# yongxuUSTC/DNN-for-speech-enhancement

Hardware: AMD Instinct MI355X
Metric: training frames/sec (257x11 input, 3x2048 DNN) (higher is better)
Workload: dtype f32; 1 GPU; C2: 2827->2048->2048->2048->257 ReLU+dropout(0.1/0.2), fp32, 256 frames/GPU/step (global bunch 256), lrate 1, momentum 0.5, 102400-frame chunk resident in HBM; parallelism=dp1, global_bunch=256, exchange=none, launcher=single process

## Files before the change

dnn-for-speech-enhancement_amd/csrc/bp_kernels.h:

```cpp
#pragma once
#include <hip/hip_runtime.h>
#include <stddef.h>
#include <stdint.h>

#include "bp_device.h"

enum { EPI_FWD_HIDDEN = 0, EPI_FWD_OUT = 1, EPI_DGRAD = 2, EPI_WGRAD_UPDATE = 3, EPI_WGRAD_STORE = 4,
       EPI_OUT_SPLIT = 6 ,
       EPI_FWD_OUT_LOGI = 7, EPI_OUT_SPLIT_LOGI = 8 };
static constexpr bool epi_out(int epi) { return epi == EPI_FWD_OUT || epi == EPI_FWD_OUT_LOGI; }
static constexpr bool epi_out_split(int epi) { return epi == EPI_OUT_SPLIT || epi == EPI_OUT_SPLIT_LOGI; }
static constexpr int OUT_SPLITS = 4;

struct GemmArgs {
    const float *A, *B;
    int lda, ldb;
    int K;
    int tiles_m, tiles_n;
#ifdef BP_TRACE
    unsigned long long *trace;
#endif
    int k_split;
    size_t slab_stride;
    float *ks_slab; unsigned *ks_ticket;
};

struct EpiArgs {
    float *C; int ldc;
    int m_limit, n_limit;
    int n_true;
    const float *bias;
    float alpha;
    int act;
    const float *aux; int ldaux;
    int lin_cols;
    float *aux2; int ldaux2;
    union {
        float scale;
        float rdiv;
    };
    float mom, c1, wc, ndiv;
    float *bias_w, *bias_d, *bias_g;
    uint32_t drop_thresh, seed_lo, seed_hi, step, layer;
    int frame_off;
    const uint8_t *mask; int ldmask;
    int loss;
    unsigned *done;
};
static_assert(sizeof(EpiArgs) == 160 && offsetof(EpiArgs, aux2) == 56 && offsetof(EpiArgs, done) == 152, "lin_cols / loss must sit in padding");
static_assert(offsetof(EpiArgs, rdiv) == 68 && offsetof(EpiArgs, scale) == 68 && offsetof(EpiArgs, mom) == 72 && offsetof(EpiArgs, ndiv) == 84,
              "rdiv lies in scale's word, in front of mom, c1, wc, ndiv");
typedef __attribute__((address_space(1))) const float *GlobalOperand;
#define BP_PIN_OPERANDS(g, ...) do { GlobalOperand pa_ = (GlobalOperand)(g).A, pb_ = (GlobalOperand)(g).B;                                \
        asm volatile("" : "+s"(pa_), "+s"(pb_), "+s"((g).lda), "+s"((g).ldb), "+s"((g).K), "+s"((g).tiles_m), "+s"((g).tiles_n), ##__VA_ARGS__); \
        (g).A = (const float *)pa_; (g).B = (const float *)pb_; } while (0)
__device__ __forceinline__ GemmArgs operand_args(const GemmArgs &s)
{
    GemmArgs g{};
    g.A = s.A; g.B = s.B; g.lda = s.lda; g.ldb = s.ldb; g.K = s.K; g.tiles_m = s.tiles_m; g.tiles_n = s.tiles_n;
    return g;
}

struct EpiPre { float bias; f32x16 p0, p1; };

template <class T>
__device__ __forceinline__ T *uniform_ptr(T *p)
{
    const unsigned long long v = (unsigned long long)p;
    const unsigned lo = __builtin_amdgcn_readfirstlane((unsigned)v), hi = __builtin_amdgcn_readfirstlane((unsigned)(v >> 32));
    typedef __attribute__((address_space(1))) T *GlobalPtr;
    return (T *)(GlobalPtr)(((unsigned long long)hi << 32) | lo);
}

template <class T>
__device__ __forceinline__ T *sgpr_row_base(T *p)
{
    typedef __attribute__((address_space(1))) T *GlobalPtr;
    GlobalPtr q = (GlobalPtr)p;
    asm volatile("" : "+s"(q));
    return (T *)q;
}

template <int EPI, int R0, int RN>
__device__ __forceinline__ void epilogue_fetch(const EpiArgs &e, int mb, int nb, int lane, EpiPre &p)
{
    if constexpr (EPI == EPI_WGRAD_UPDATE) {
        const int mbc = mb < e.m_limit ? mb : 0;
        const float *cw = uniform_ptr(e.C + (size_t)mbc * e.ldc + nb);
        const float *cd = uniform_ptr(e.aux2 + (size_t)mbc * e.ldc + nb);
        const unsigned ldc = __builtin_amdgcn_readfirstlane(e.ldc);
        const unsigned lob = 4u * ((unsigned)(4 * (lane >> 5)) * (unsigned)e.ldc + (unsigned)(lane & 31));
#pragma unroll
        for (int r = R0; r < R0 + RN; ++r) {
            const unsigned ro = (unsigned)((r & 3) + 8 * (r >> 2)) * ldc;
            p.p0[r] = *reinterpret_cast<const float *>(reinterpret_cast<const char *>(sgpr_row_base(cw + ro)) + lob);
            p.p1[r] = *reinterpret_cast<const float *>(reinterpret_cast<const char *>(sgpr_row_base(cd + ro)) + lob);
        }
        return;
    }
    const int n = nb + (lane & 31);
    const int rbase = mb + 4 * (lane >> 5);
    static_assert(!epi_out_split(EPI), "fetched as EPI_FWD_OUT[_LOGI]");
    if constexpr (EPI == EPI_FWD_HIDDEN || epi_out(EPI)) p.bias = e.bias[n];
    if constexpr (epi_out(EPI) || EPI == EPI_DGRAD) {
        if (epi_out(EPI) && !e.C) return;
#pragma unroll
        for (int r = R0; r < R0 + RN; ++r) {
            const int m = rbase + (r & 3) + 8 * (r >> 2);
            const int mc = m < e.m_limit ? m : e.m_limit - 1;
            p.p0[r] = e.aux[(size_t)mc * e.ldaux + n];
        }
    }
}

template <int R0, int RN>
__device__ __forceinline__ void block_store(const EpiArgs &e, int mb, int nb, int lane, const float (&v)[RN])
{
    if (mb + 32 <= e.m_limit) {
        float *c = uniform_ptr(e.C + (size_t)mb * e.ldc + nb);
        const unsigned ldc = __builtin_amdgcn_readfirstlane(e.ldc);
        const unsigned lob = 4u * ((unsigned)(4 * (lane >> 5)) * (unsigned)e.ldc + (unsigned)(lane & 31));
#pragma unroll
        for (int r = R0; r < R0 + RN; ++r) {
            const unsigned ro = (unsigned)((r & 3) + 8 * (r >> 2)) * ldc;
            *reinterpret_cast<float *>(reinterpret_cast<char *>(sgpr_row_base(c + ro)) + lob) = v[r - R0];
        }
        return;
    }
    const int n = nb + (lane & 31), rbase = mb + 4 * (lane >> 5);
#pragma unroll
    for (int r = R0; r < R0 + RN; ++r) {
        const int m = rbase + (r & 3) + 8 * (r >> 2);
        if (m < e.m_limit) e.C[(size_t)m * e.ldc + n] = v[r - R0];
    }
}

template <int EPI, int R0, int RN, bool RCP = false>
__device__ __forceinline__ void epilogue_block(const EpiArgs &e, int mb, int nb, const f32x16 &acc, int lane,
                                               const EpiPre &p)
{
    static_assert(!RCP || EPI == EPI_WGRAD_UPDATE, "only the fused update divides");
    static_assert(RN % 4 == 0 && R0 % 4 == 0, "register range must cover whole 4-row groups");
    if constexpr (EPI == EPI_WGRAD_UPDATE || EPI == EPI_WGRAD_STORE) {
        const int n = nb + (lane & 31);
        if (n >= e.n_limit || mb >= e.m_limit) return;
        float *cw = uniform_ptr(e.C + (size_t)mb * e.ldc + nb);
        const unsigned ldc = __builtin_amdgcn_readfirstlane(e.ldc);
        const unsigned lob = 4u * ((unsigned)(4 * (lane >> 5)) * (unsigned)e.ldc + (unsigned)(lane & 31));
#pragma unroll
        for (int r = R0; r < R0 + RN; ++r) {
            const unsigned ro = (unsigned)((r & 3) + 8 * (r >> 2)) * ldc;
            if constexpr (EPI == EPI_WGRAD_UPDATE) {
                float *cd = uniform_ptr(e.aux2 + (size_t)mb * e.ldc + nb);
                const float w = p.p0[r];
                const float d = update_delta<RCP>(e.mom, e.c1, e.wc, e.ndiv, e.rdiv, p.p1[r], acc[r], w);
                *reinterpret_cast<float *>(reinterpret_cast<char *>(sgpr_row_base(cd + ro)) + lob) = d;
                *reinterpret_cast<float *>(reinterpret_cast<char *>(sgpr_row_base(cw + ro)) + lob) = d + 1.0f * w;
            } else {
                __hip_atomic_store(reinterpret_cast<float *>(reinterpret_cast<char *>(sgpr_row_base(cw + ro)) + lob), acc[r], __ATOMIC_RELAXED, __HIP_MEMORY_SCOPE_SYSTEM);
            }
        }
        return;
    }
    const int n = nb + (lane & 31);
    const int rbase = mb + 4 * (lane >> 5);
    if (n >= e.n_limit) return;
    if constexpr (EPI == EPI_FWD_HIDDEN) {
        const float bn = p.bias;
        const bool live = n < e.n_true;
        float y[RN];
#pragma unroll
        for (int q = R0 / 4; q < (R0 + RN) / 4; ++q) {
            uint32_t w[4] = {0xFFFFFFFFu, 0xFFFFFFFFu, 0xFFFFFFFFu, 0xFFFFFFFFu};
            const int r0 = rbase + 8 * q;
            if (e.mask) {
#pragma unroll
                for (int j = 0; j < 4; ++j) w[j] = (r0 + j < e.m_limit && live && e.mask[(size_t)(r0 + j) * e.ldmask + n]) ? 0u : 0xFFFFFFFFu;
            } else if (e.drop_thresh) drop_words4(w, r0, n, e.frame_off, (uint32_t)e.n_true, e.layer, e.step, e.seed_lo, e.seed_hi);
#pragma unroll
            for (int j = 0; j < 4; ++j) {
                y[q * 4 + j - R0] = act_fwd(e.act, e.alpha * acc[q * 4 + j] + bn);
                if (!live || w[j] < e.drop_thresh) y[q * 4 + j - R0] = 0.0f;
            }
        }
        block_store<R0, RN>(e, mb, nb, lane, y);
    } else if constexpr (EPI == EPI_FWD_OUT) {
        const float bn = p.bias;
        const bool live = n < e.n_true;
#pragma unroll
        for (int r = R0; r < R0 + RN; ++r) {
            const int m = rbase + (r & 3) + 8 * (r >> 2);
            if (m < e.m_limit) {
                const float o = live ? e.alpha * acc[r] + bn : 0.0f;
                if (e.aux2) e.aux2[(size_t)m * e.ldaux2 + n] = o;
                if (e.C) e.C[(size_t)m * e.ldc + n] = live ? e.scale * (o - p.p0[r]) : 0.0f;
            }
        }
    } else if constexpr (EPI == EPI_FWD_OUT_LOGI) {
        const float bn = p.bias;
        const bool live = n < e.n_true, logi = live && n >= e.lin_cols, chain = logi && e.loss == 1;
#pragma unroll
        for (int r = R0; r < R0 + RN; ++r) {
            const int m = rbase + (r & 3) + 8 * (r >> 2);
            if (m < e.m_limit) {
                const float z = live ? e.alpha * acc[r] + bn : 0.0f;
                const float o = logi ? 1.0f / (1.0f + expf(-z)) : z;
                if (e.aux2) e.aux2[(size_t)m * e.ldaux2 + n] = o;
                if (e.C) {
                    float d = live ? e.scale * (o - p.p0[r]) : 0.0f;
                    if (chain) d *= o * (1.0f - o);
                    e.C[(size_t)m * e.ldc + n] = d;
                }
            }
        }
    } else if constexpr (EPI == EPI_DGRAD) {
        float d[RN];
#pragma unroll
        for (int r = R0; r < R0 + RN; ++r) d[r - R0] = act_bwd(e.act, p.p0[r]) * acc[r];
        block_store<R0, RN>(e, mb, nb, lane, d);
    } else {
        static_assert(EPI == EPI_WGRAD_UPDATE || EPI == EPI_WGRAD_STORE, "epilogue without a branch");
    }
}

template <bool RCP>
__device__ __forceinline__ void bias_update(const EpiArgs &e, int n, float s)
{
    const float d = update_delta<RCP>(e.mom, e.c1, 0.0f, e.ndiv, e.rdiv, e.bias_d[n], s, e.bias_w[n]);
    e.bias_d[n] = d;
    e.bias_w[n] = d + 1.0f * e.bias_w[n];
}

template <int R0>
__device__ __forceinline__ void out_split_store(const EpiArgs &e, float *slab, int mb, int nb, const f32x16 &acc, int lane)
{
    const int n = nb + (lane & 31), rbase = mb + 4 * (lane >> 5);
    if (n >= e.n_limit) return;
#pragma unroll
    for (int r = R0; r < R0 + 4; ++r) {
        const int m = rbase + (r & 3) + 8 * (r >> 2);
        if (m < e.m_limit) __hip_atomic_store(slab + (size_t)m * e.ldc + n, acc[r], __ATOMIC_RELAXED, __HIP_MEMORY_SCOPE_AGENT);
    }
}
template <int R0>
__device__ __forceinline__ void out_split_sum(const EpiArgs &e, const float *slab0, size_t stride, int mb, int nb, f32x16 &acc, int lane)
{
    const int n = nb + (lane & 31), rbase = mb + 4 * (lane >> 5);
    if (n >= e.n_limit) return;
    float p[OUT_SPLITS][4];
#pragma unroll
    for (int z = 0; z < OUT_SPLITS; ++z)
#pragma unroll
        for (int rr = 0; rr < 4; ++rr) {
            const int r = R0 + rr, m = rbase + (r & 3) + 8 * (r >> 2), mc = m < e.m_limit ? m : e.m_limit - 1;
            p[z][rr] = __hip_atomic_load(slab0 + z * stride + (size_t)mc * e.ldc + n, __ATOMIC_RELAXED, __HIP_MEMORY_SCOPE_AGENT);
        }
#pragma unroll
    for (int rr = 0; rr < 4; ++rr) {
        float s = p[0][rr];
#pragma unroll
        for (int z = 1; z < OUT_SPLITS; ++z) s += p[z][rr];
        acc[R0 + rr] = s;
    }
}

template <int KS, int KSI>
__device__ __forceinline__ void ksplit_give(const f32x16 &acc, float *red, int wq, int lane)
{
    constexpr int RN = 16 / KS;
#pragma unroll
    for (int o = 0; o < KS; ++o) {
        if (o == KSI) continue;
#pragma unroll
        for (int rr = 0; rr < RN; ++rr) red[(((wq * KS + o) * KS + KSI) * RN + rr) * 64 + lane] = acc[o * RN + rr];
    }
}
template <int KS, int KSI>
__device__ __forceinline__ void ksplit_take(f32x16 &acc, const float *red, int wq, int lane)
{
    constexpr int RN = 16 / KS;
#pragma unroll
    for (int src = 0; src < KS; ++src) {
        if (src == KSI) continue;
#pragma unroll
        for (int rr = 0; rr < RN; ++rr) acc[KSI * RN + rr] += red[(((wq * KS + KSI) * KS + src) * RN + rr) * 64 + lane];
    }
}

template <int NVA, int NVB>
struct TileRegs { float4 a[NVA]; float4 b[NVB]; };

template <int BM, int BN, int BK, int WM, int WN, bool A_KC, bool B_KC, int EPI>
struct GemmCfg {
    static constexpr int KS = 4 / (WM * WN);
    static constexpr int TM = BM / (WM * 32), TN = BN / (WN * 32);
    static constexpr int LDA_S = A_KC ? BM + 1 : BM;
    static constexpr int LDB_S = B_KC ? BN + 1 : BN;
    static constexpr int A_STAGE = (BK * LDA_S + 3) & ~3, B_STAGE = (BK * LDB_S + 3) & ~3;
    static constexpr int NVA = BM * BK / 4 / 256, NVB = BN * BK / 4 / 256;
    static constexpr int LPS = (BK / 4 < 8) ? BK / 4 : 8;
    static constexpr bool BIASG = (EPI == EPI_WGRAD_UPDATE || EPI == EPI_WGRAD_STORE);
    static_assert(WM * WN * KS == 4 && TM >= 1 && TN >= 1, "wave layout");
    static_assert(BK % (2 * KS) == 0 && BK % 4 == 0, "BK");
    static_assert(NVA >= 1 && NVB >= 1, "tile too small for 256 threads");
    using Regs = TileRegs<NVA, NVB>;

    static constexpr int NCH = (TM * TN == 1) ? 2 : 1;
    static constexpr int NK = BK / KS / 2;
    static constexpr int step_row(int ks, int s) { return ks * (BK / KS) + 2 * s; }
    static constexpr int step_chain(int s) { return s % NCH; }

    struct Offs { unsigned a[NVA]; unsigned b[NVB]; };
    static __device__ __forceinline__ unsigned lane_off(unsigned &off)
    {
        asm volatile("" : "+v"(off));
        return off;
    }
    static __device__ __forceinline__ void make_offs(Offs &o, const GemmArgs &g, int tid)
    {
#pragma unroll
        for (int i = 0; i < NVA; ++i) {
            const int f = tid + i * 256;
            if constexpr (A_KC) {
                const int l8 = f % LPS, seg = f / LPS, row = seg % BM, k4 = (seg / BM) * LPS + l8;
                o.a[i] = 4u * (unsigned)(row * g.lda + k4 * 4);
            } else {
                const int c4 = f % (BM / 4), k = f / (BM / 4);
                o.a[i] = 4u * (unsigned)(k * g.lda + c4 * 4);
            }
        }
#pragma unroll
        for (int i = 0; i < NVB; ++i) {
            const int f = tid + i * 256;
            if constexpr (B_KC) {
                const int l8 = f % LPS, seg = f / LPS, row = seg % BN, k4 = (seg / BN) * LPS + l8;
                o.b[i] = 4u * (unsigned)(row * g.ldb + k4 * 4);
            } else {
                const int c4 = f % (BN / 4), k = f / (BN / 4);
                o.b[i] = 4u * (unsigned)(k * g.ldb + c4 * 4);
            }
        }
    }
    static __device__ __forceinline__ const float *base_a(const GemmArgs &g, int m0, int k0)
    {
        return A_KC ? g.A + (size_t)m0 * g.lda + k0 : g.A + (size_t)k0 * g.lda + m0;
    }
    static __device__ __forceinline__ const float *base_b(const GemmArgs &g, int n0, int k0)
    {
        return B_KC ? g.B + (size_t)n0 * g.ldb + k0 : g.B + (size_t)k0 * g.ldb + n0;
    }
    static __device__ __forceinline__ void load_a(Regs &r, int i, const float *pa, Offs &o)
    {
        r.a[i] = *reinterpret_cast<const float4 *>(reinterpret_cast<const char *>(pa) + lane_off(o.a[i]));
    }
    static __device__ __forceinline__ void load_b(Regs &r, int i, const float *pb, Offs &o)
    {
        r.b[i] = *reinterpret_cast<const float4 *>(reinterpret_cast<const char *>(pb) + lane_off(o.b[i]));
    }
    static __device__ __forceinline__ void load(Regs &r, const float *pa, const float *pb, Offs &o)
    {
#pragma unroll
        for (int i = 0; i < NVA; ++i) load_a(r, i, pa, o);
#pragma unroll
        for (int i = 0; i < NVB; ++i) load_b(r, i, pb, o);
    }

    static __device__ __forceinline__ void store_a(const Regs &r, int i, float *As, int tid, int krows)
    {
        const int f = tid + i * 256;
        float4 v = r.a[i];
        if constexpr (BIASG && !A_KC) {
            if (f / (BM / 4) >= krows) v = make_float4(0.f, 0.f, 0.f, 0.f);
        }
        if constexpr (A_KC) {
            const int l8 = f % LPS, seg = f / LPS, row = seg % BM, k4 = (seg / BM) * LPS + l8;
            As[(k4 * 4 + 0) * LDA_S + row] = v.x; As[(k4 * 4 + 1) * LDA_S + row] = v.y;
            As[(k4 * 4 + 2) * LDA_S + row] = v.z; As[(k4 * 4 + 3) * LDA_S + row] = v.w;
        } else {
            const int c4 = f % (BM / 4), k = f / (BM / 4);
            *reinterpret_cast<float4 *>(As + k * LDA_S + c4 * 4) = v;
        }
    }
    static __device__ __forceinline__ void store_b(const Regs &r, int i, float *Bs, int tid, float4 &bsum)
    {
        const int f = tid + i * 256;
        const float4 v = r.b[i];
        if constexpr (B_KC) {
            const int l8 = f % LPS, seg = f / LPS, row = seg % BN, k4 = (seg / BN) * LPS + l8;
            Bs[(k4 * 4 + 0) * LDB_S + row] = v.x; Bs[(k4 * 4 + 1) * LDB_S + row] = v.y;
            Bs[(k4 * 4 + 2) * LDB_S + row] = v.z; Bs[(k4 * 4 + 3) * LDB_S + row] = v.w;
        } else {
            const int c4 = f % (BN / 4), k = f / (BN / 4);
            *reinterpret_cast<float4 *>(Bs + k * LDB_S + c4 * 4) = v;
            if constexpr (BIASG) {
                bsum.x += v.x; bsum.y += v.y; bsum.z += v.z; bsum.w += v.w;
            }
        }
    }
    static __device__ __forceinline__ void store(const Regs &r, float *As, float *Bs, int tid, float4 &bsum, int krows)
    {
#pragma unroll
        for (int i = 0; i < NVA; ++i) store_a(r, i, As, tid, krows);
#pragma unroll
        for (int i = 0; i < NVB; ++i) store_b(r, i, Bs, tid, bsum);
    }

    template <bool DO_STORE, bool DO_LOAD>
    static __device__ __forceinline__ void step(const float *As, const float *Bs, f32x16 (&acc)[NCH][TM][TN], int ks,
                                                int a_off, int b_off, int kh, const Regs &rs, float *AsN, float *BsN,
                                                Regs &rl, const float *pa, const float *pb, Offs &o, int tid,
                                                float4 &bsum, int krows)
    {
        constexpr int NP = NVA + NVB, RD = NK < 4 ? NK : 4;
        const float *ap = As + (step_row(ks, 0) + kh) * LDA_S + a_off;
        const float *bp = Bs + (step_row(ks, 0) + kh) * LDB_S + b_off;
        float av[NK][TM], bv[NK][TN];
        __builtin_amdgcn_sched_barrier(0);
#pragma unroll
        for (int s = 0; s < RD; ++s) {
#pragma unroll
            for (int i = 0; i < TM; ++i) av[s][i] = ap[step_row(0, s) * LDA_S + i * 32];
#pragma unroll
            for (int j = 0; j < TN; ++j) bv[s][j] = bp[step_row(0, s) * LDB_S + j * 32];
        }
        __builtin_amdgcn_sched_barrier(0);
        int pl = 0, ps = 0;
#pragma unroll
        for (int s = 0; s < NK; ++s) {
#pragma unroll
            for (int i = 0; i < TM; ++i)
#pragma unroll
                for (int j = 0; j < TN; ++j)
                    acc[step_chain(s)][i][j] = __builtin_amdgcn_mfma_f32_32x32x2f32(av[s][i], bv[s][j], acc[step_chain(s)][i][j], 0, 0, 0);
            if (s + RD < NK) {
#pragma unroll
                for (int i = 0; i < TM; ++i) av[s + RD][i] = ap[step_row(0, s + RD) * LDA_S + i * 32];
#pragma unroll
                for (int j = 0; j < TN; ++j) bv[s + RD][j] = bp[step_row(0, s + RD) * LDB_S + j * 32];
            }
            if constexpr (DO_LOAD) {
#pragma unroll
                for (int q = 0; q < NP; ++q) {
                    if (q == pl && (q * NK) / NP == s) {
                        if (q < NVA) load_a(rl, q, pa, o); else load_b(rl, q - NVA, pb, o);
                        ++pl;
                    }
                }
            }
            if constexpr (DO_STORE) {
#pragma unroll
                for (int q = 0; q < NP; ++q) {
                    if (q == ps && (q * NK) / NP == s) {
                        if (q < NVA) store_a(rs, q, AsN, tid, krows); else store_b(rs, q - NVA, BsN, tid, bsum);
                        ++ps;
                    }
                }
            }
            __builtin_amdgcn_sched_barrier(0);
        }
    }
};

template <bool M_SLOW>
__device__ __forceinline__ void xcd_tile(int b, int tiles_m, int tiles_n, int &tile_m, int &tile_n)
{
    if ((tiles_n & 7) == 0) {
        const int xcd = b & 7, j = b >> 3, per = tiles_n >> 3;
        if constexpr (M_SLOW) { tile_n = xcd * per + j % per; tile_m = j / per; }
        else { tile_n = xcd * per + j / tiles_m; tile_m = j % tiles_m; }
    } else { tile_m = b % tiles_m; tile_n = b / tiles_m; }
}
template <class Multi>
__device__ __forceinline__ int problem_of(const Multi &a, int b, int p)
{
    while (p + 1 < a.n && b >= a.first_tile[p + 1]) ++p;
    return p;
}

static inline bool covers_tiles(long long workgroups, const GemmArgs &g, int slices = 1)
{
    return g.tiles_m >= 0 && g.tiles_n >= 0 && workgroups >= (long long)g.tiles_m * g.tiles_n * slices;
}
template <class Multi>
static inline bool multi_covers_tiles(const Multi &a)
{
    if (a.n < 1 || a.n > 4) return false;
    for (int p = 0; p < a.n; ++p)
        if (!covers_tiles((long long)a.first_tile[p + 1] - a.first_tile[p], a.g[p])) return false;
    return true;
}

template <int BM, int BN, int BK, int WM, int WN, bool A_KC, bool B_KC, int EPI>
struct GemmKernel {
    using Cfg = GemmCfg<BM, BN, BK, WM, WN, A_KC, B_KC, EPI>;
    static constexpr int KS = Cfg::KS, TM = Cfg::TM, TN = Cfg::TN;
    static constexpr int A_STAGE = Cfg::A_STAGE, B_STAGE = Cfg::B_STAGE, STAGE = A_STAGE + B_STAGE;
    static constexpr bool BIASG = Cfg::BIASG;
    static constexpr int RED = (KS > 1) ? KS * WM * WN * 16 * 64 : 0;
    static constexpr int BIASRED = BIASG ? 256 / (BN / 4) * BN : 0;
    static constexpr int SMEM0 = (2 * STAGE > RED) ? 2 * STAGE : RED;
    static constexpr int SMEM = SMEM0 > BIASRED ? SMEM0 : BIASRED;
    static constexpr int MIN_WG = (SMEM * 4 > 80 * 1024) ? 1 : 2;

static __device__ __forceinline__ void run(const GemmArgs &g_in, const EpiArgs &e_in, int b, int block_y, float *smem)
{
    using Regs = typename Cfg::Regs;
    const int tid = threadIdx.x, lane = tid & 63, wave = __builtin_amdgcn_readfirstlane(tid >> 6);
    constexpr int EPI_E = EPI == EPI_OUT_SPLIT ? EPI_FWD_OUT : EPI == EPI_OUT_SPLIT_LOGI ? EPI_FWD_OUT_LOGI : EPI;
#ifdef BP_TRACE
#define TRACE(i) do { if (tid == 0 && g_in.trace) { g_in.trace[(size_t)b * 8 + (i)] = wall_clock64();           \
        if ((i) == 0) g_in.trace[(size_t)b * 8 + 6] = clock64();              \
        if ((i) == 3) g_in.trace[(size_t)b * 8 + 7] = clock64();           \
    } } while (0)
#else
#define TRACE(i) ((void)0)
#endif
#define K0_OF(t) (((t) * BK) < last_k0 ? ((t) * BK) : last_k0)
#define PA(t) Cfg::base_a(g, m0, K0_OF(t))
#define PB(t) Cfg::base_b(g, n0, K0_OF(t))
#define AS(buf) (smem + (buf) * STAGE)
#define BS(buf) (smem + (buf) * STAGE + A_STAGE)

    TRACE(0);
    GemmArgs g = operand_args(g_in);
    if constexpr (epi_out_split(EPI)) {
        const size_t kz = (size_t)block_y * g_in.k_split;
        g.A += A_KC ? kz : kz * g.lda;
        g.B += B_KC ? kz : kz * g.ldb;
    }
    BP_PIN_OPERANDS(g);
    const int tiles = g.tiles_m * g.tiles_n;
    if (b >= tiles) return;
    const int nt = (g.K + BK - 1) / BK, last_k0 = (nt - 1) * BK;
    typename Cfg::Offs offs;
    Cfg::make_offs(offs, g, tid);
    int tile_m, tile_n;
    xcd_tile<BIASG>(b, g.tiles_m, g.tiles_n, tile_m, tile_n);
    const int m0 = tile_m * BM, n0 = tile_n * BN;
    Regs r0, r1;
    Cfg::load(r0, PA(0), PB(0), offs);
    Cfg::load(r1, PA(1), PB(1), offs);
    __builtin_amdgcn_sched_barrier(0);

    int behind = 0;
    asm volatile("" : "+s"(behind));
    const EpiArgs e = *reinterpret_cast<const EpiArgs *>(reinterpret_cast<const char *>(&e_in) + behind);
    const int ks = wave / (WM * WN), wq = wave % (WM * WN), wm = wq / WN, wn = wq % WN;
    const int a_off = wm * TM * 32 + (lane & 31), b_off = wn * TN * 32 + (lane & 31);
    const int kh = lane >> 5;

    float4 bsum = make_float4(0.f, 0.f, 0.f, 0.f);
    const bool do_bias = BIASG && tile_m == 0;

    constexpr int NCH = Cfg::NCH;
    f32x16 accs[NCH][TM][TN];
#pragma unroll
    for (int c = 0; c < NCH; ++c)
#pragma unroll
        for (int i = 0; i < TM; ++i)
#pragma unroll
            for (int j = 0; j < TN; ++j)
#pragma unroll
                for (int r = 0; r < 16; ++r) accs[c][i][j][r] = 0.0f;

    EpiPre pre[TM][TN];
    const int mb0 = m0 + wm * TM * 32, nb0 = n0 + wn * TN * 32;
    if constexpr (KS == 1) {
#pragma unroll
        for (int i = 0; i < TM; ++i)
#pragma unroll
            for (int j = 0; j < TN; ++j) epilogue_fetch<EPI_E, 0, 16>(e, mb0 + i * 32, nb0 + j * 32, lane, pre[i][j]);
    } else {
        static_assert(KS == 1 || (TM == 1 && TN == 1), "in-workgroup k-split needs one block per wave");
        if (ks == 0) epilogue_fetch<EPI_E, 0, 16 / KS>(e, mb0, nb0, lane, pre[0][0]);
        if (ks == 1) epilogue_fetch<EPI_E, 16 / KS, 16 / KS>(e, mb0, nb0, lane, pre[0][0]);
        if constexpr (KS == 4) {
            if (ks == 2) epilogue_fetch<EPI_E, 8, 4>(e, mb0, nb0, lane, pre[0][0]);
            if (ks == 3) epilogue_fetch<EPI_E, 12, 4>(e, mb0, nb0, lane, pre[0][0]);
        }
    }

#define STEP(ST, LD, buf, RS, TS, RL, TL)                                                                  \
    Cfg::template step<ST, LD>(AS(buf), BS(buf), accs, ks, a_off, b_off, kh, RS, AS((buf) ^ 1), BS((buf) ^ 1),    \
                               RL, PA(TL), PB(TL), offs, tid, bsum, g.K - (TS) * BK)
    Cfg::store(r0, AS(0), BS(0), tid, bsum, g.K);
    __syncthreads();
    TRACE(1);
    int t = 0, buf = 0;
    if (__builtin_expect(nt >= 3, 1))
    for (; t + 3 <= nt; t += 2) {
        STEP(true, true, 0, r1, t + 1, r0, t + 2);
        __syncthreads();
        STEP(true, true, 1, r0, t + 2, r1, t + 3);
        __syncthreads();
    }
    if (nt - t == 2) {
        STEP(true, false, 0, r1, t + 1, r0, 0);
        __syncthreads();
        buf = 1;
    }
    STEP(false, false, buf, r0, 0, r0, 0);
    __syncthreads();
    TRACE(2);
#undef STEP
    __builtin_amdgcn_s_waitcnt(0x0F70);
    f32x16 (&acc)[TM][TN] = accs[0];
    if constexpr (NCH == 2) {
#pragma unroll
        for (int i = 0; i < TM; ++i)
#pragma unroll
            for (int j = 0; j < TN; ++j)
#pragma unroll
                for (int r = 0; r < 16; ++r) acc[i][j][r] += accs[1][i][j][r];
    }

    if constexpr (KS > 1) {
        if (ks == 0) ksplit_give<KS, 0>(acc[0][0], smem, wq, lane);
        if (ks == 1) ksplit_give<KS, 1>(acc[0][0], smem, wq, lane);
        if constexpr (KS == 4) {
            if (ks == 2) ksplit_give<KS, 2>(acc[0][0], smem, wq, lane);
            if (ks == 3) ksplit_give<KS, 3>(acc[0][0], smem, wq, lane);
        }
        __syncthreads();
        if (ks == 0) ksplit_take<KS, 0>(acc[0][0], smem, wq, lane);
        if (ks == 1) ksplit_take<KS, 1>(acc[0][0], smem, wq, lane);
        if constexpr (KS == 4) {
            if (ks == 2) ksplit_take<KS, 2>(acc[0][0], smem, wq, lane);
            if (ks == 3) ksplit_take<KS, 3>(acc[0][0], smem, wq, lane);
        }
        if constexpr (BIASG) __syncthreads();
    }

    if constexpr (BIASG && !B_KC) {
        if (do_bias) {
            constexpr int CG = BN / 4, RG = 256 / CG;
            float *red = smem;
            const int c4 = tid % CG, rg = tid / CG;
            *reinterpret_cast<float4 *>(red + rg * BN + c4 * 4) = bsum;
            __syncthreads();
            if (tid < BN && (n0 + tid) < e.n_limit) {
                float s = 0.f;
#pragma unroll
                for (int r = 0; r < RG; ++r) s += red[r * BN + tid];
                const int n = n0 + tid;
                if constexpr (EPI == EPI_WGRAD_UPDATE) {
                    if (e.rdiv != 0.0f) bias_update<true>(e, n, s); else bias_update<false>(e, n, s);
                } else {
                    e.bias_g[n] = s;
                }
            }
        }
    }

    bool finish = true;
    if constexpr (epi_out_split(EPI)) {
        static_assert(KS == 4 && OUT_SPLITS == 4, "one 32x32 block per workgroup, four registers of it per wave");
        float *mine = g_in.ks_slab + (size_t)block_y * g_in.slab_stride;
        if (ks == 0) out_split_store<0>(e, mine, mb0, nb0, acc[0][0], lane);
        if (ks == 1) out_split_store<4>(e, mine, mb0, nb0, acc[0][0], lane);
        if (ks == 2) out_split_store<8>(e, mine, mb0, nb0, acc[0][0], lane);
        if (ks == 3) out_split_store<12>(e, mine, mb0, nb0, acc[0][0], lane);
        finish = last_arrival(g_in.ks_ticket + b, reinterpret_cast<unsigned *>(smem), OUT_SPLITS);
        if (finish) {
            if (ks == 0) out_split_sum<0>(e, g_in.ks_slab, g_in.slab_stride, mb0, nb0, acc[0][0], lane);
            if (ks == 1) out_split_sum<4>(e, g_in.ks_slab, g_in.slab_stride, mb0, nb0, acc[0][0], lane);
            if (ks == 2) out_split_sum<8>(e, g_in.ks_slab, g_in.slab_stride, mb0, nb0, acc[0][0], lane);
            if (ks == 3) out_split_sum<12>(e, g_in.ks_slab, g_in.slab_stride, mb0, nb0, acc[0][0], lane);
        }
    }

    if constexpr (EPI == EPI_WGRAD_UPDATE) {
        static_assert(KS == 1, "the update runs on whole blocks");
        if (e.rdiv != 0.0f) {
#pragma unroll
            for (int i = 0; i < TM; ++i)
#pragma unroll
                for (int j = 0; j < TN; ++j)
                    epilogue_block<EPI_E, 0, 16, true>(e, mb0 + i * 32, nb0 + j * 32, acc[i][j], lane, pre[i][j]);
        } else {
#pragma unroll
            for (int i = 0; i < TM; ++i)
#pragma unroll
                for (int j = 0; j < TN; ++j)
                    epilogue_block<EPI_E, 0, 16, false>(e, mb0 + i * 32, nb0 + j * 32, acc[i][j], lane, pre[i][j]);
        }
    } else if constexpr (KS == 1) {
#pragma unroll
        for (int i = 0; i < TM; ++i)
#pragma unroll
            for (int j = 0; j < TN; ++j)
                epilogue_block<EPI_E, 0, 16>(e, mb0 + i * 32, nb0 + j * 32, acc[i][j], lane, pre[i][j]);
    } else if (finish) {
        if (ks == 0) epilogue_block<EPI_E, 0, 16 / KS>(e, mb0, nb0, acc[0][0], lane, pre[0][0]);
        if (ks == 1) epilogue_block<EPI_E, 16 / KS, 16 / KS>(e, mb0, nb0, acc[0][0], lane, pre[0][0]);
        if constexpr (KS == 4) {
            if (ks == 2) epilogue_block<EPI_E, 8, 4>(e, mb0, nb0, acc[0][0], lane, pre[0][0]);
            if (ks == 3) epilogue_block<EPI_E, 12, 4>(e, mb0, nb0, acc[0][0], lane, pre[0][0]);
        }
    }
    TRACE(3);
#undef K0_OF
#undef PA
#undef PB
#undef AS
#undef BS
#undef TRACE
}
};

template <int BM, int BN, int BK, int WM, int WN, bool A_KC, bool B_KC, int EPI, int TAG = 0>
__global__ __launch_bounds__(256, (GemmKernel<BM, BN, BK, WM, WN, A_KC, B_KC, EPI>::MIN_WG)) void bp_gemm(const GemmArgs g, const EpiArgs e)
{
    using K = GemmKernel<BM, BN, BK, WM, WN, A_KC, B_KC, EPI>;
    __shared__ __attribute__((aligned(16))) float smem[K::SMEM];
    K::run(g, e, blockIdx.x, blockIdx.y, smem);
}

struct MultiArgs {
    GemmArgs g[4];
    EpiArgs e[4];
    int first_tile[5];
    int n;
};
#ifndef BP_TRACE
static_assert(sizeof(MultiArgs) == 920 && offsetof(MultiArgs, first_tile) == 896 && offsetof(MultiArgs, n) == 916, "MultiArgs layout");
#endif
template <class K>
__global__ __launch_bounds__(256, K::MIN_WG) void bp_gemm_multi(const MultiArgs a)
{
    __shared__ __attribute__((aligned(16))) float smem[K::SMEM];
    const int b = blockIdx.x;
    int n = a.n, first = a.first_tile[0], next = a.first_tile[1];
    GemmArgs g = a.g[0];
    BP_PIN_OPERANDS(g, "+s"(n), "+s"(first), "+s"(next));
    int p = 0;
    if (n > 1 && b >= next) {
        asm volatile("");
        p = problem_of(a, b, 1);
        g = a.g[p];
        first = a.first_tile[p]; next = a.first_tile[p + 1];
    }
    K::run(g, a.e[p], b - first, 0, smem);
}

struct StageArgs {
    float *x; int ld, width;
    const float *fea; int fea_dim, win;
    const float *nat; const int *win_start, *nat_row;
    int rows; uint32_t thresh; int frame_off; uint32_t seed_lo, seed_hi, step;
    float *t; int ldt, twidth; const float *targ_frames; const int *targ_frame;
    int yb_in;
    int nbx;
};
__device__ __forceinline__ void stage_rows_block(const StageArgs &a, int bx, int by, int tx)
{
    const int r0 = bx * 4, c = (by * 256 + tx) * 4;
    if (c >= a.ld) return;
    float4 v[4];
#pragma unroll
    for (int j = 0; j < 4; ++j)
        v[j] = *reinterpret_cast<const float4 *>(a.fea + (size_t)(r0 + j < a.rows ? r0 + j : a.rows - 1) * a.fea_dim + c);
    if (a.thresh) {
        uint32_t drop = 0;
#pragma unroll 1
        for (int k = 0; k < 4; ++k) {
            if (c + k >= a.width) break;
            uint32_t w[4];
            drop_words4(w, r0, c + k, a.frame_off, (uint32_t)a.width, 0u, a.step, a.seed_lo, a.seed_hi);
            const uint32_t m = (w[0] < a.thresh ? 1u : 0u) | (w[1] < a.thresh ? 2u : 0u) | (w[2] < a.thresh ? 4u : 0u) | (w[3] < a.thresh ? 8u : 0u);
            drop |= m << (4 * k);
        }
#pragma unroll
        for (int j = 0; j < 4; ++j) {
            if (drop & (1u << (0 + j))) v[j].x = 0.0f;
            if (drop & (1u << (4 + j))) v[j].y = 0.0f;
            if (drop & (1u << (8 + j))) v[j].z = 0.0f;
            if (drop & (1u << (12 + j))) v[j].w = 0.0f;
        }
    }
#pragma unroll
    for (int j = 0; j < 4; ++j) if (r0 + j < a.rows) *reinterpret_cast<float4 *>(a.x + (size_t)(r0 + j) * a.ld + c) = v[j];
}
__device__ __forceinline__ void stage_block(const StageArgs &a, int bx, int by, int tx)
{
    if (!a.win_start) { stage_rows_block(a, bx, by, tx); return; }
    const int r0 = bx * 4;
    float v[4] = {0.0f, 0.0f, 0.0f, 0.0f};
    int rr[4];
#pragma unroll
    for (int j = 0; j < 4; ++j) rr[j] = r0 + j < a.rows ? r0 + j : a.rows - 1;
    if (by >= a.yb_in) {
        const int c = (by - a.yb_in) * 256 + tx;
        if (c >= a.ldt) return;
        if (c < a.twidth) {
            int tf[4];
#pragma unroll
            for (int j = 0; j < 4; ++j) tf[j] = a.targ_frame[rr[j]];
#pragma unroll
            for (int j = 0; j < 4; ++j) v[j] = a.targ_frames[(size_t)tf[j] * a.twidth + c];
        }
#pragma unroll
        for (int j = 0; j < 4; ++j) if (r0 + j < a.rows) a.t[(size_t)(r0 + j) * a.ldt + c] = v[j];
        return;
    }
    const int c = by * 256 + tx;
    if (c >= a.ld) return;
    if (c < a.win) {
        int ws[4];
#pragma unroll
        for (int j = 0; j < 4; ++j) ws[j] = a.win_start[rr[j]];
#pragma unroll
        for (int j = 0; j < 4; ++j) v[j] = a.fea[(size_t)ws[j] * a.fea_dim + c];
    } else if (c < a.width) {
        int nr[4];
#pragma unroll
        for (int j = 0; j < 4; ++j) nr[j] = a.nat_row[rr[j]];
#pragma unroll
        for (int j = 0; j < 4; ++j) v[j] = a.nat[(size_t)nr[j] * a.fea_dim + (c - a.win)];
    }
    uint32_t w[4] = {~0u, ~0u, ~0u, ~0u};
    if (a.thresh && c < a.width) drop_words4(w, r0, c, a.frame_off, (uint32_t)a.width, 0u, a.step, a.seed_lo, a.seed_hi);
#pragma unroll
    for (int j = 0; j < 4; ++j) if (r0 + j < a.rows) a.x[(size_t)(r0 + j) * a.ld + c] = w[j] < a.thresh ? 0.0f : v[j];
}
__global__ __launch_bounds__(256) void bp_stage_bunch(const StageArgs a)
{
    stage_block(a, blockIdx.x % a.nbx, blockIdx.x / a.nbx, threadIdx.x);
}

__global__ void bp_apply_mask(const float *in, float *out, int ld, int width, const uint8_t *mask, int n_frames)
{
    const int u = blockIdx.x * blockDim.x + threadIdx.x, f = blockIdx.y;
    if (u >= ld || f >= n_frames) return;
    float v = in[(size_t)f * ld + u];
    if (u < width && mask[(size_t)f * width + u]) v = 0.0f;
    out[(size_t)f * ld + u] = v;
}

__global__ void bp_fill_normal(float *buf, int ld, int width, int rows, uint32_t seed_lo, uint32_t seed_hi,
                               uint32_t stream)
{
    const size_t i = (size_t)blockIdx.x * blockDim.x + threadIdx.x;
    const size_t per_row = (size_t)(ld / 4);
    if (i >= per_row * (size_t)rows) return;
    const size_t r = i / per_row; const int c = (int)(i % per_row) * 4;
    uint32_t w0 = (uint32_t)i, w1 = (uint32_t)(i >> 32), w2 = stream, w3 = 0x5EEDu;
    philox4x32_10(w0, w1, w2, w3, seed_lo, seed_hi);
    const float u0 = (w0 + 1.0f) * 2.3283064365386963e-10f, u1 = w1 * 2.3283064365386963e-10f;
    const float u2 = (w2 + 1.0f) * 2.3283064365386963e-10f, u3 = w3 * 2.3283064365386963e-10f;
    const float r0 = sqrtf(-2.0f * logf(fminf(u0, 1.0f))), r1 = sqrtf(-2.0f * logf(fminf(u2, 1.0f)));
    float v[4] = { r0 * cosf(6.283185307179586f * u1), r0 * sinf(6.283185307179586f * u1),
                   r1 * cosf(6.283185307179586f * u3), r1 * sinf(6.283185307179586f * u3) };
    float4 o;
    o.x = (c + 0 < width) ? v[0] : 0.f; o.y = (c + 1 < width) ? v[1] : 0.f;
    o.z = (c + 2 < width) ? v[2] : 0.f; o.w = (c + 3 < width) ? v[3] : 0.f;
    *reinterpret_cast<float4 *>(buf + r * ld + c) = o;
}

template <class K>
__global__ __launch_bounds__(256, K::MIN_WG) void bp_out_split_stage(const GemmArgs g, const EpiArgs e, int n_gemm, const StageArgs st)
{
    __shared__ __attribute__((aligned(16))) float smem[K::SMEM];
    const int b = blockIdx.x;
    GemmArgs gg = g;
    int ng = n_gemm;
    BP_PIN_OPERANDS(gg, "+s"(ng), "+s"(gg.k_split));
    if (b < ng) { const int tiles = gg.tiles_m * gg.tiles_n; K::run(gg, e, b % tiles, b / tiles, smem); }
    else { const int i = b - ng; stage_block(st, i % st.nbx, i / st.nbx, threadIdx.x); }
}
```

Before: 1.341 million frames/s.

## Move tile barrier inside GEMM step and prefetch next tile's LDS fragments early

The workgroup barrier between K-tiles moves from after each step into the step itself, placed after the last LDS fragment read of the current tile (one step earlier when A is K-contiguous and B is not). Right after the barrier, the first fragments of the next tile are read from the freshly stored buffer and carried into the next step in registers. Stores into the next buffer are spread over the slots before the barrier. The aim is to hide the barrier wait and the LDS read latency of the next tile's start behind the remaining MFMAs of the current tile. In exchange it holds more live registers for the carried fragments and compresses the store schedule, which could raise register pressure or LDS contention.

```diff
diff --git a/dnn-for-speech-enhancement_amd/csrc/bp_kernels.h b/dnn-for-speech-enhancement_amd/csrc/bp_kernels.h
--- a/dnn-for-speech-enhancement_amd/csrc/bp_kernels.h
+++ b/dnn-for-speech-enhancement_amd/csrc/bp_kernels.h
@@ -309,6 +309,14 @@
     static constexpr int NK = BK / KS / 2;
     static constexpr int step_row(int ks, int s) { return ks * (BK / KS) + 2 * s; }
     static constexpr int step_chain(int s) { return s % NCH; }
+    static constexpr bool EARLY_BAR = A_KC && !B_KC;
+    static constexpr int NP = NVA + NVB;
+    static constexpr int RD = NK < 4 ? NK : 4;
+    static constexpr int LAST_READ = NK - RD - 1;
+    static constexpr int BAR = (EARLY_BAR && NK > RD + 2) ? NK - 2 : NK - 1;
+    static constexpr int store_slot(int q) { return (q * (BAR + 1)) / NP; }
+    static constexpr int load_slot(int q) { return (q * NK) / NP; }
+    static_assert(BAR > LAST_READ && BAR <= NK - 1, "the barrier's wait covers every fragment read of the tile, none of them young");
 
     struct Offs { unsigned a[NVA]; unsigned b[NVB]; };
     static __device__ __forceinline__ unsigned lane_off(unsigned &off)
@@ -405,13 +413,25 @@
         for (int i = 0; i < NVB; ++i) store_b(r, i, Bs, tid, bsum);
     }
 
+    struct Frags { float a[RD][TM], b[RD][TN]; };
+    static __device__ __forceinline__ void read_first(Frags &f, const float *As, const float *Bs, int ks, int a_off, int b_off, int kh)
+    {
+        const float *ap = As + (step_row(ks, 0) + kh) * LDA_S + a_off;
+        const float *bp = Bs + (step_row(ks, 0) + kh) * LDB_S + b_off;
+#pragma unroll
+        for (int s = 0; s < RD; ++s) {
+#pragma unroll
+            for (int i = 0; i < TM; ++i) f.a[s][i] = ap[step_row(0, s) * LDA_S + i * 32];
+#pragma unroll
+            for (int j = 0; j < TN; ++j) f.b[s][j] = bp[step_row(0, s) * LDB_S + j * 32];
+        }
+    }
     template <bool DO_STORE, bool DO_LOAD>
     static __device__ __forceinline__ void step(const float *As, const float *Bs, f32x16 (&acc)[NCH][TM][TN], int ks,
                                                 int a_off, int b_off, int kh, const Regs &rs, float *AsN, float *BsN,
                                                 Regs &rl, const float *pa, const float *pb, Offs &o, int tid,
-                                                float4 &bsum, int krows)
-    {
-        constexpr int NP = NVA + NVB, RD = NK < 4 ? NK : 4;
+                                                float4 &bsum, int krows, Frags &f)
+    {
         const float *ap = As + (step_row(ks, 0) + kh) * LDA_S + a_off;
         const float *bp = Bs + (step_row(ks, 0) + kh) * LDB_S + b_off;
         float av[NK][TM], bv[NK][TN];
@@ -419,11 +439,10 @@
 #pragma unroll
         for (int s = 0; s < RD; ++s) {
 #pragma unroll
-            for (int i = 0; i < TM; ++i) av[s][i] = ap[step_row(0, s) * LDA_S + i * 32];
-#pragma unroll
-            for (int j = 0; j < TN; ++j) bv[s][j] = bp[step_row(0, s) * LDB_S + j * 32];
-        }
-        __builtin_amdgcn_sched_barrier(0);
+            for (int i = 0; i < TM; ++i) av[s][i] = f.a[s][i];
+#pragma unroll
+            for (int j = 0; j < TN; ++j) bv[s][j] = f.b[s][j];
+        }
         int pl = 0, ps = 0;
 #pragma unroll
         for (int s = 0; s < NK; ++s) {
@@ -432,6 +451,7 @@
 #pragma unroll
                 for (int j = 0; j < TN; ++j)
                     acc[step_chain(s)][i][j] = __builtin_amdgcn_mfma_f32_32x32x2f32(av[s][i], bv[s][j], acc[step_chain(s)][i][j], 0, 0, 0);
+            if (s == 0) __builtin_amdgcn_sched_barrier(0);
             if (s + RD < NK) {
 #pragma unroll
                 for (int i = 0; i < TM; ++i) av[s + RD][i] = ap[step_row(0, s + RD) * LDA_S + i * 32];
@@ -441,7 +461,7 @@
             if constexpr (DO_LOAD) {
 #pragma unroll
                 for (int q = 0; q < NP; ++q) {
-                    if (q == pl && (q * NK) / NP == s) {
+                    if (q == pl && load_slot(q) == s) {
                         if (q < NVA) load_a(rl, q, pa, o); else load_b(rl, q - NVA, pb, o);
                         ++pl;
                     }
@@ -450,10 +470,15 @@
             if constexpr (DO_STORE) {
 #pragma unroll
                 for (int q = 0; q < NP; ++q) {
-                    if (q == ps && (q * NK) / NP == s) {
+                    if (q == ps && store_slot(q) == s) {
                         if (q < NVA) store_a(rs, q, AsN, tid, krows); else store_b(rs, q - NVA, BsN, tid, bsum);
                         ++ps;
                     }
+                }
+                if (s == BAR) {
+                    __syncthreads();
+                    __builtin_amdgcn_sched_barrier(0);
+                    read_first(f, AsN, BsN, ks, a_off, b_off, kh);
                 }
             }
             __builtin_amdgcn_sched_barrier(0);
@@ -582,21 +607,20 @@
 
 #define STEP(ST, LD, buf, RS, TS, RL, TL)                                                                  \
     Cfg::template step<ST, LD>(AS(buf), BS(buf), accs, ks, a_off, b_off, kh, RS, AS((buf) ^ 1), BS((buf) ^ 1),    \
-                               RL, PA(TL), PB(TL), offs, tid, bsum, g.K - (TS) * BK)
+                               RL, PA(TL), PB(TL), offs, tid, bsum, g.K - (TS) * BK, frags)
     Cfg::store(r0, AS(0), BS(0), tid, bsum, g.K);
     __syncthreads();
     TRACE(1);
+    typename Cfg::Frags frags;
+    Cfg::read_first(frags, AS(0), BS(0), ks, a_off, b_off, kh);
     int t = 0, buf = 0;
     if (__builtin_expect(nt >= 3, 1))
     for (; t + 3 <= nt; t += 2) {
         STEP(true, true, 0, r1, t + 1, r0, t + 2);
-        __syncthreads();
         STEP(true, true, 1, r0, t + 2, r1, t + 3);
-        __syncthreads();
     }
     if (nt - t == 2) {
         STEP(true, false, 0, r1, t + 1, r0, 0);
-        __syncthreads();
         buf = 1;
     }
     STEP(false, false, buf, r0, 0, r0, 0);
```

Result: faster. 1.359 million frames/s, median of 6 (+1.4%).
